# xarray-contrib/xeofs

Hardware: AMD Instinct MI355X
Metric: EOF randomized-SVD GB/s (algorithmic: 16 passes x n x p x 4 B per fit / fit time) (higher is better)
Workload: dtype f32 data, split-fp16 MFMA (f16x3+f16x3), f32 accumulate

## Files before the change

include/eofx.h:

```cpp
#ifndef EOFX_H
#define EOFX_H

#include <stdint.h>

#ifdef __cplusplus
extern "C" {
#endif

#define EOFX_ABI_VERSION 1
#define EOFX_MAX_SKETCH 256

#define EOFX_OK 0
#define EOFX_ERR_ARG (-1)
#define EOFX_ERR_HIP (-2)
#define EOFX_ERR_PARTIAL_NAN (-3)
#define EOFX_ERR_NAN_MISMATCH (-4)
#define EOFX_ERR_RANK (-5)
#define EOFX_ERR_LINALG (-6)
#define EOFX_ERR_NOMEM (-7)
#define EOFX_ERR_SHAPE (-8)

typedef struct eofx_ctx eofx_ctx;
typedef struct eofx_mat eofx_mat;

// ... 91 lines not shown
                           int n_oversamples, int n_iter, const float *omega, int flip, float *Q1,
                           float *s, float *Q2, float *scores1, float *scores2, float *norm1,
                           float *norm2, double *tsc);
typedef const float *(*eofx_sketch_fn)(void *user);
int eofx_crosscov_rsvd_lazy_f32(eofx_ctx *ctx, const eofx_mat *x, const eofx_mat *y, int k, int n_oversamples,
                                int n_iter, eofx_sketch_fn omega_fn, void *omega_user, int flip, float *Q1, float *s,
                                float *Q2, float *scores1, float *scores2, float *norm1, float *norm2, double *tsc);

int eofx_panel_tmul_f32(eofx_ctx *ctx, const eofx_mat *m, const float *Zn, float *Yp, int L,
                        int precision);
int eofx_panel_mul_f32(eofx_ctx *ctx, const eofx_mat *m, const float *Yp, float *Wn, int L,
                       int precision);
int eofx_panel_gram_f64(eofx_ctx *ctx, const float *P, int64_t rows_pad, int L, double *G);
int eofx_panel_cholqr_f32(eofx_ctx *ctx, const float *P, int64_t rows_pad, int L, int l,
                          const double *G, float *out);
int eofx_panel_rinv_f64(eofx_ctx *ctx, const double *G, int L, int l, double *Rinv);
int eofx_panel_matmul_f32(eofx_ctx *ctx, const float *P, int64_t rows_pad, int L,
                          const double *M, int Lo, float *out);
int eofx_panel_colminmax_f32(eofx_ctx *ctx, const float *P, int64_t rows, int L, float *mx,
                             float *mn);
int eofx_panel_export_f32(eofx_ctx *ctx, const float *P, int64_t rows, int L, int k,
                          const double *sign, float *dst);
int eofx_panel_import_f32(eofx_ctx *ctx, const float *src, int64_t rows, int l, float *P,
                          int64_t rows_pad, int L);

int eofx_hilbert_f32(eofx_ctx *ctx, const eofx_mat *a, int padding, double decay_factor,
                     eofx_mat **out_imag, eofx_mat **out_real);
int eofx_mat_sumsq_f64(eofx_ctx *ctx, const eofx_mat *m, double *out);
int eofx_panel_rownorm_f64(eofx_ctx *ctx, const float *P, int64_t rows, int L, double *out);
int eofx_mat_feature_norms_f64(eofx_ctx *ctx, const eofx_mat *m, double *out);
// ... 79 lines not shown
```

xeofs_amd/_lib.py:

```python

from __future__ import annotations

import ctypes as C
import os

import numpy as np

_HERE = os.path.dirname(os.path.abspath(__file__))
LIB_PATH = os.environ.get("EOFX_LIB") or os.path.join(_HERE, "lib", "libeofx.so")

EOFX_OK = 0
ERR_ARG, ERR_HIP, ERR_PARTIAL_NAN, ERR_NAN_MISMATCH, ERR_RANK, ERR_LINALG, ERR_NOMEM, ERR_SHAPE = (
    -1, -2, -3, -4, -5, -6, -7, -8)

_vp = C.c_void_p
_i64 = C.c_int64
_int = C.c_int
_pi64 = C.POINTER(C.c_int64)
_pd = C.POINTER(C.c_double)

SKETCH_FN = C.CFUNCTYPE(C.c_void_p, C.c_void_p)

ALLREDUCE_FN = C.CFUNCTYPE(C.c_int, C.c_void_p, C.c_void_p, C.c_int64, C.c_int, C.c_int, C.c_void_p)

# ... 15 lines not shown
    "eofx_mat_from_dense_f32": (_int, [_vp, _vp, _i64, _i64, _i64, C.POINTER(_vp)]),
    "eofx_mat_destroy": (_int, [_vp, _vp]),
    "eofx_mat_shape": (_int, [_vp, _pi64, _pi64, _pi64, _pi64]),
    "eofx_mat_download_f32": (_int, [_vp, _vp, _vp]),
    "eofx_rsvd_f32": (_int, [_vp, _vp, _int, _int, _int, _vp, _int, _vp, _vp, _vp]),
    "eofx_project_f32": (_int, [_vp, _vp, _vp, _int, _vp]),
    "eofx_reconstruct_f32": (_int, [_vp, _vp, _vp, _i64, _i64, _int, _vp]),
    "eofx_crosscov_rsvd_f32": (_int, [_vp, _vp, _vp, _int, _int, _int, _vp, _int, _vp, _vp, _vp, _vp,
                                      _vp, _vp, _vp, _pd]),
    "eofx_crosscov_rsvd_lazy_f32": (_int, [_vp, _vp, _vp, _int, _int, _int, SKETCH_FN, _vp, _int, _vp, _vp, _vp, _vp,
                                           _vp, _vp, _vp, _pd]),
    "eofx_panel_tmul_f32": (_int, [_vp, _vp, _vp, _vp, _int, _int]),
    "eofx_panel_mul_f32": (_int, [_vp, _vp, _vp, _vp, _int, _int]),
    "eofx_panel_gram_f64": (_int, [_vp, _vp, _i64, _int, _vp]),
    "eofx_panel_cholqr_f32": (_int, [_vp, _vp, _i64, _int, _int, _vp, _vp]),
    "eofx_panel_rinv_f64": (_int, [_vp, _vp, _int, _int, _vp]),
    "eofx_panel_matmul_f32": (_int, [_vp, _vp, _i64, _int, _vp, _int, _vp]),
    "eofx_panel_colminmax_f32": (_int, [_vp, _vp, _i64, _int, _vp, _vp]),
    "eofx_panel_export_f32": (_int, [_vp, _vp, _i64, _int, _int, _vp, _vp]),
    "eofx_panel_import_f32": (_int, [_vp, _vp, _i64, _int, _vp, _i64, _int]),
    "eofx_hilbert_f32": (_int, [_vp, _vp, _int, C.c_double, C.POINTER(_vp), C.POINTER(_vp)]),
    "eofx_mat_sumsq_f64": (_int, [_vp, _vp, _pd]),
    "eofx_fit_f32": (_int, [_vp, _vp, _i64, _i64, _int, _int, _vp, _int, _int, _int, _int, _vp, _i64, _int,
                            C.POINTER(_vp), _vp, _vp, _vp, _vp, _pi64, _pi64, _pd, _vp, _vp, _vp, C.POINTER(C.c_int)]),
    "eofx_fit_first_f32": (_int, [_vp, _vp, _i64, _i64, _int, _int, _vp, _int, _vp, _int, _int, _vp, C.POINTER(_vp),
                                  _vp, _vp, _vp, _vp, _pi64, _pi64, _pd, C.POINTER(C.c_int)]),
    "eofx_ctx_fit_info": (_int, [_vp, _pd]),
    "eofx_ctx_last_iterations": (_int, [_vp, C.POINTER(_int)]),
    "eofx_comm_unique_id": (_int, [C.c_char_p]),
    "eofx_ctx_comm_init_rccl": (_int, [_vp, C.c_char_p, _int, _int]),
# ... 117 lines not shown
```

xeofs_amd/csrc/eofx_abi.hip:

```cpp
#include <chrono>
#include "eofx_hfft.hpp"
#include "eofx_kernels.hpp"
#include "eofx_fit.hpp"
#include "eofx_gram.hpp"
#include "eofx_axb_dma.hpp"
#include "eofx_hosteig.hpp"
#include "eofx_hostla.hpp"
#include "eofx_lag.hpp"
#include "eofx_gw.hpp"
#include "eofx_spca.hpp"
#include "eofx_lagcov.hpp"
#include "eofx_lowpass.hpp"
#include "eofx_pcmul.hpp"
#include "eofx_viewcov.hpp"
#include "eofx_lrfill.hpp"
#include "eofx_plans.hpp"
#include "eofx_sketch.hpp"
#include "eofx_hilbert_host.hpp"
#include "eofx_gwplan.hpp"
#ifndef EOFX_AXB_DMA_DEFAULT
#define EOFX_AXB_DMA_DEFAULT 1
#endif

#include <algorithm>
// ... 708 lines not shown
  }
  if (plan.S > 1) {
    const int64_t count4 = rows_pad * L / 4;
    hipLaunchKernelGGL(splitk_reduce_kernel, dim3((int)std::min<int64_t>((count4 + 255) / 256, amax_out ? 2048 : 4096)), dim3(256), 0,
                       ctx->stream, out, W, count4, plan.S, amax_out);
    KCHK();
  }
  return EOFX_OK;
}

static int launch_gram(eofx_ctx* ctx, const float* P, int64_t rows, int L, double* G) {
  const int nb = (L + 63) / 64;
  const int nbx = gram_parts(rows, L);
  ArenaScope scope(ctx);
  ARENA(double, part, (size_t)nbx * L * L);
  hipLaunchKernelGGL(gram_mfma_kernel, dim3(nbx, nb * nb), dim3(256), 0, ctx->stream, P, rows, L, part);
  KCHK();
  const int64_t count = (int64_t)L * L;
  hipLaunchKernelGGL(f64_reduce_kernel, dim3((int)((count + 63) / 64)), dim3(256), 0, ctx->stream,
                     part, G, count, nbx);
  KCHK();
  return EOFX_OK;
}
static int launch_matmul(eofx_ctx* ctx, const float* P, int64_t rows, int L, const double* Mx, int Lo,
                         float* out, bool upper = false) {
  int KW = (int)std::min<int64_t>(round_up(L, 64), 256);
  if (L > 256) {
    static const int kw_env = std::getenv("EOFX_PMM_KW") ? atoi(std::getenv("EOFX_PMM_KW")) : 0;
    if (kw_env == 128 || kw_env == 256) KW = kw_env;
  }
  const size_t smem = (size_t)KW * PMM_LD * sizeof(double);
  if (smem > 64 * 1024)
    HIPCHK(hipFuncSetAttribute(reinterpret_cast<const void*>(panel_matmul_kernel<false>), hipFuncAttributeMaxDynamicSharedMemorySize, (int)smem));
  const int64_t units = (rows + 127) / 128;
  const int64_t gx = L <= KW ? std::min<int64_t>(units, 1024) : units;
  dim3 grid((int)std::max<int64_t>(1, gx), (Lo + 63) / 64);
  hipLaunchKernelGGL(panel_matmul_kernel<false>, grid, dim3(256), smem, ctx->stream, P, rows, L, Mx, Lo, out, KW, amax_new(ctx, out),
                     (int64_t)0, (int64_t)0, 1, (const float*)nullptr, upper ? 1 : 0);
  KCHK();
  return EOFX_OK;
}
static int launch_matmul_gen(eofx_ctx* ctx, const float* P, int64_t ldp, int64_t slab, int cpb, int64_t rows, int L, const double* Mx, int Lo,
                             const float* sub, float* out) {
  const int KW = (int)std::min<int64_t>(round_up(L, 64), 256);
  const size_t smem = (size_t)KW * PMM_LD * sizeof(double);
  if (smem > 64 * 1024)
    HIPCHK(hipFuncSetAttribute(reinterpret_cast<const void*>(panel_matmul_kernel<true>), hipFuncAttributeMaxDynamicSharedMemorySize, (int)smem));
  const int64_t units = (rows + 127) / 128;
  const int64_t gx = L <= KW ? std::min<int64_t>(units, 1024) : units;
  dim3 grid((int)std::max<int64_t>(1, gx), (Lo + 63) / 64);
  hipLaunchKernelGGL(panel_matmul_kernel<true>, grid, dim3(256), smem, ctx->stream, P, rows, L, Mx, Lo, out, KW, amax_new(ctx, out), ldp,
                     slab, cpb, sub);
  KCHK();
// ... 7 lines not shown
  KCHK();
  const int64_t count = (int64_t)La * Lb;
  hipLaunchKernelGGL(f64_reduce_kernel, dim3((int)((count + 63) / 64)), dim3(256), 0, ctx->stream, part, C, count, nbx);
  KCHK();
  return EOFX_OK;
}

static int launch_rinv(eofx_ctx* ctx, const double* G, int L, int l, double* Rinv);
static size_t matmul_nt_scratch(eofx_ctx* ctx, int64_t rows, int L, int Lo);
static int launch_matmul_nt(eofx_ctx* ctx, const float* P, int64_t rows, int L, const double* Mx, int Lo, float* out);
static int launch_cholqr(eofx_ctx* ctx, const float* P, int64_t rows, int L, int l, const double* G,
                         float* out) {
  ArenaScope scope(ctx);
  ARENA(double, Rinv, (size_t)L * L);
  CHK(launch_rinv(ctx, G, L, l, Rinv));
  return launch_matmul(ctx, P, rows, L, Rinv, L, out, true);
}

static int launch_colminmax(eofx_ctx* ctx, const float* P, int64_t rows, int L, float* mx, float* mn) {
  const int nparts = (int)std::max<int64_t>(1, std::min<int64_t>((rows + 127) / 128, 1024));
  ArenaScope scope(ctx);
  ARENA(float, pmx, (size_t)nparts * L);
  ARENA(float, pmn, (size_t)nparts * L);
  hipLaunchKernelGGL(colminmax_part_kernel, dim3(nparts, (L + 63) / 64), dim3(256), 0, ctx->stream, P,
                     rows, L, pmx, pmn);
  KCHK();
  hipLaunchKernelGGL(colminmax_final_kernel, dim3((L + 63) / 64), dim3(256), 0, ctx->stream, pmx, pmn,
                     nparts, L, mx, mn);
  KCHK();
  return EOFX_OK;
}
// ... 806 lines not shown
  return panel_mul(ctx, m, Yp, Wn, L, prec);
}
extern "C" int eofx_panel_gram_f64(eofx_ctx* ctx, const float* P, int64_t rows_pad, int L, double* G) {
  if (!ctx || !P || !G || L % 32) return set_err(ctx, EOFX_ERR_ARG, "bad argument");
  ENTER(ctx);
  CHK(arena_reserve(ctx, (size_t)(4 * gram_parts(rows_pad, L) + 1) * L * L * sizeof(double)));
  return launch_gram(ctx, P, rows_pad, L, G);
}
extern "C" int eofx_panel_cholqr_f32(eofx_ctx* ctx, const float* P, int64_t rows_pad, int L, int l,
                                     const double* G, float* out) {
  if (!ctx || !P || !G || !out || P == out) return set_err(ctx, EOFX_ERR_ARG, "bad argument");
  ENTER(ctx);
  CHK(arena_reserve(ctx, (size_t)2 * L * L * sizeof(double) + (l > 64 ? rinv_blocked_bytes(l) : 0)));
  return launch_cholqr(ctx, P, rows_pad, L, l, G, out);
}
extern "C" int eofx_panel_rinv_f64(eofx_ctx* ctx, const double* G, int L, int l, double* Rinv) {
  if (!ctx || !G || !Rinv || L <= 0 || l <= 0 || l > L || G == Rinv) return set_err(ctx, EOFX_ERR_ARG, "bad argument");
  ENTER(ctx);
  if (l > 64) CHK(arena_reserve(ctx, rinv_blocked_bytes(l)));
  return launch_rinv(ctx, G, L, l, Rinv);
}
extern "C" int eofx_panel_matmul_f32(eofx_ctx* ctx, const float* P, int64_t rows_pad, int L,
                                     const double* M, int Lo, float* out) {
  if (!ctx || !P || !M || !out || P == out) return set_err(ctx, EOFX_ERR_ARG, "bad argument");
  ENTER(ctx);
  if (matmul_nt_ok(rows_pad, L, Lo)) {
    const size_t need = matmul_nt_scratch(ctx, rows_pad, L, Lo);
    if (need && arena_reserve(ctx, need) == EOFX_OK) return launch_matmul_nt(ctx, P, rows_pad, L, M, Lo, out);
  }
  return launch_matmul(ctx, P, rows_pad, L, M, Lo, out);
// ... 27 lines not shown
struct LinOp {
  int64_t tall, small, tall_pad, small_pad;
  std::function<int(const float*, float*, int, int)> fwd;
  std::function<int(const float*, float*, int, int)> bwd;
  std::function<int(double*, int64_t)> reduce_tall_gram;
  std::function<int(double*, int64_t)> reduce_small_gram;
  int64_t rule_tall_pad = 0;
};

struct RsvdOut {
  float* Tvec;
  float* Svec;
  int Lo;
  std::vector<double> s;
  int64_t tall_pad = 0, small_pad = 0;
};

extern "C" int eofx_orth_tall_rule(int64_t tall_rows_pad, int L, int prec_power) {
  return orth_tall_rule(tall_rows_pad, L, prec_power) ? 1 : 0;
}
extern "C" int eofx_peaked_spectrum(const double* G, int ld, int l) {
  if (!G || l <= 0) return 0;
  std::vector<double> A((size_t)l * l), w(l), V((size_t)l * l);
  for (int i = 0; i < l; ++i)
    for (int j = 0; j < l; ++j) A[(size_t)i * l + j] = 0.5 * (G[(size_t)i * ld + j] + G[(size_t)j * ld + i]);
  for (double v : A)
    if (!std::isfinite(v)) return 0;
  if (eofx_host_eigh_f64(A.data(), l, w.data(), V.data()) != EOFX_OK) return 1;
  if (!(w[0] > 0.0)) return 0;
  return hostla::peaked_spectrum(w.data(), l) ? 1 : 0;
// ... 155 lines not shown
        rc = set_err(ctx, EOFX_ERR_HIP, "asynchronous Gram download failed");
        break;
      }
      peaked_pending = true;
    }
    rc = launch_cholqr(ctx, Ws, op.small_pad, L, l, ask ? G0 : G, Zs);
  }
  if (peaked_ev) {
    if (peaked_pending) (void)hipEventSynchronize(peaked_ev);
    (void)hipEventDestroy(peaked_ev);
  }
  if (rc != EOFX_OK) return rc;
  if (range) CHK((*range)(Zs, Yt, L));
  else CHK(fwd(Zs, Yt, pp));
  CHK(gram_tall(Yt, G));
  CHK(launch_cholqr(ctx, Yt, op.tall_pad, L, l, G, Qt));
  CHK(gram_tall(Qt, G));
  CHK(launch_rinv(ctx, G, L, l, R2));
  CHK(op.bwd(Qt, Zs, L, pf));
  CHK(launch_matmul(ctx, Zs, op.small_pad, L, R2, L, Ws));
  CHK(gram_small(Ws, G));
  double* hG = pin;
  double* hR2 = pin + (size_t)L * L;
  HIPCHK(hipMemcpyAsync(hG, G, sizeof(double) * L * L, hipMemcpyDeviceToHost, ctx->stream));
  HIPCHK(hipMemcpyAsync(hR2, R2, sizeof(double) * L * L, hipMemcpyDeviceToHost, ctx->stream));
  HIPCHK(hipStreamSynchronize(ctx->stream));
  std::vector<double> Gl((size_t)l * l), w(l), Uh((size_t)l * l);
  for (int i = 0; i < l; ++i)
    for (int j = 0; j < l; ++j) {
      const double v = 0.5 * (hG[(size_t)i * L + j] + hG[(size_t)j * L + i]);
      if (!std::isfinite(v))
        return set_err(ctx, EOFX_ERR_LINALG,
// ... 8 lines not shown
    const double sv = std::sqrt(std::max(w[j], 0.0));
    out.s[j] = sv;
    invs[j] = sv > 0.0 ? 1.0 / sv : 0.0;
  }
  for (int i = 0; i < l; ++i) {
    double* m1 = &M1[(size_t)i * Lo];
    for (int q = 0; q < l; ++q) {
      const double r = hR2[(size_t)i * L + q];
      const double* uq = &Uh[(size_t)q * l];
      for (int j = 0; j < k; ++j) m1[j] += r * uq[j];
    }
    for (int j = 0; j < k; ++j) M2[(size_t)i * Lo + j] = Uh[(size_t)i * l + j] * invs[j];
  }
  HIPCHK(hipMemcpyAsync(Md, M1.data(), sizeof(double) * L * Lo, hipMemcpyHostToDevice, ctx->stream));
  HIPCHK(hipMemcpyAsync(Md2, M2.data(), sizeof(double) * L * Lo, hipMemcpyHostToDevice, ctx->stream));
  CHK(launch_matmul(ctx, Qt, op.tall_pad, L, Md, Lo, Tv));
  CHK(launch_matmul(ctx, Ws, op.small_pad, L, Md2, Lo, Sv));
  HIPCHK(hipStreamSynchronize(ctx->stream));
  out.Tvec = Tv;
  out.Svec = Sv;
  out.Lo = Lo;
  out.tall_pad = op.tall_pad;
  out.small_pad = op.small_pad;
  return EOFX_OK;
}

static int comm_allreduce(eofx_ctx* ctx, void* buf, int64_t count, int dtype, int op);
static int sign_rule(eofx_ctx* ctx, const float* Vpanel, int64_t rows, int Lo, int k,
                     std::vector<double>& sign, bool over_ranks = false) {
  ArenaScope scope(ctx);
  ARENA(float, mx, 2 * (size_t)Lo);
  float* mn = mx + Lo;
  CHK(launch_colminmax(ctx, Vpanel, rows, Lo, mx, mn));
  if (over_ranks) {
    hipLaunchKernelGGL(negate_kernel, dim3(1), dim3(256), 0, ctx->stream, mn, Lo);
    KCHK();
    CHK(comm_allreduce(ctx, mx, 2 * (int64_t)Lo, 0, 1));
  }
  std::vector<float> hmx(Lo), hmn(Lo);
  HIPCHK(hipMemcpyAsync(hmx.data(), mx, sizeof(float) * Lo, hipMemcpyDeviceToHost, ctx->stream));
  HIPCHK(hipMemcpyAsync(hmn.data(), mn, sizeof(float) * Lo, hipMemcpyDeviceToHost, ctx->stream));
  HIPCHK(hipStreamSynchronize(ctx->stream));
  sign.assign(k, 1.0);
  for (int j = 0; j < k; ++j) sign[j] = (std::fabs(hmx[j]) >= std::fabs(hmn[j])) ? 1.0 : -1.0;
  return EOFX_OK;
}

typedef std::function<int(double*, int64_t)> GramReduce;
// ... 35 lines not shown
      CHK(refill());
      continue;
    }
    HIPCHK(hipMemcpyAsync(Mx, hM.data(), sizeof(double) * Lo * Lo, hipMemcpyHostToDevice, ctx->stream));
    CHK(launch_matmul(ctx, P, rows_pad, Lo, Mx, Lo, tmp));
    HIPCHK(hipMemcpy2DAsync(P + first, sizeof(float) * Lo, tmp + first, sizeof(float) * Lo, sizeof(float) * (size_t)(k - first), (size_t)rows_pad,
                            hipMemcpyDeviceToDevice, ctx->stream));
    HIPCHK(hipStreamSynchronize(ctx->stream));
    ++rounds_done;
  }
  return EOFX_OK;
}

static int fix_null_modes(eofx_ctx* ctx, const RsvdOut& ro, int64_t tall, int64_t small, int k,
                          const GramReduce* reduce_tall = nullptr, int64_t tall_total = -1,
                          const GramReduce* reduce_small = nullptr, int64_t small_total = -1) {
  int first_null = k;
  const double s0 = ro.s.empty() ? 0.0 : ro.s[0];
  for (int j = k - 1; j >= 0 && !(ro.s[j] > 1e-5 * s0); --j) first_null = j;
  if (first_null < k && s0 >= 0.0 && std::isfinite(s0) && ro.tall_pad >= tall && ro.small_pad >= small) {
    CHK(fix_null_columns(ctx, ro.Tvec, tall, ro.tall_pad, ro.Lo, k, first_null, reduce_tall, tall_total));
    CHK(fix_null_columns(ctx, ro.Svec, small, ro.small_pad, ro.Lo, k, first_null, reduce_small, small_total));
  }
  return EOFX_OK;
}

struct FactorShards {
  const GramReduce* reduce_tall = nullptr;
  int64_t tall_total = -1;
  const GramReduce* reduce_small = nullptr;
  int64_t small_total = -1;
};
static int rsvd_finish(eofx_ctx* ctx, const RsvdOut& ro, bool right_is_tall, int64_t left_rows, int64_t right_rows, int k, int flip,
                       float* left, float* s, float* right, double s_divisor = 1.0, const FactorShards* shards = nullptr,
                       std::vector<double>* sign_out = nullptr) {
  const int64_t tall = right_is_tall ? right_rows : left_rows, small = right_is_tall ? left_rows : right_rows;
  const FactorShards local, &sh = shards ? *shards : local;
  CHK(fix_null_modes(ctx, ro, tall, small, k, sh.reduce_tall, sh.tall_total, sh.reduce_small, sh.small_total));
  const float* Rp = right_is_tall ? ro.Tvec : ro.Svec;
  const float* Lp = right_is_tall ? ro.Svec : ro.Tvec;
  std::vector<double> sign;
  if (flip) CHK(sign_rule(ctx, Rp, right_rows, ro.Lo, k, sign, shards != nullptr));
  CHK(export_panel(ctx, Lp, left_rows, ro.Lo, k, flip ? sign.data() : nullptr, left));
  CHK(export_panel(ctx, Rp, right_rows, ro.Lo, k, flip ? sign.data() : nullptr, right));
  if (s) {
    std::vector<float> hs(k);
    for (int j = 0; j < k; ++j) hs[j] = (float)(ro.s[j] / s_divisor);
    HIPCHK(hipMemcpy(s, hs.data(), sizeof(float) * k, hipMemcpyDefault));
  }
  HIPCHK(hipStreamSynchronize(ctx->stream));
  if (sign_out) sign_out->swap(sign);
  return EOFX_OK;
}

static const float* identity_sketch(int64_t small, int l, std::vector<float>& eye) {
  eye.assign((size_t)small * l, 0.f);
  for (int64_t i = 0; i < l; ++i) eye[(size_t)i * l + i] = 1.f;
// ... 3122 lines not shown
```

xeofs_amd/csrc/eofx_kernels.hpp:

```cpp
#pragma once
#include <hip/hip_runtime.h>
#include <stdint.h>

#include "eofx_mfma64.hpp"
#include "eofx_plans.hpp"

namespace eofx {

typedef float f32x16 __attribute__((ext_vector_type(16)));
typedef float f32x4 __attribute__((ext_vector_type(4)));
typedef float f32x2 __attribute__((ext_vector_type(2)));

__device__ __forceinline__ void aff_split(double sh, float& hi, float& lo) {
  hi = (float)sh;
  lo = (float)(sh - (double)hi);
}
__device__ __forceinline__ float aff_map(float x, float sh_hi, float sh_lo, float scale) {
  return ((x - sh_hi) - sh_lo) * scale;
}
__device__ __forceinline__ float aff_fma(float x, float sh_hi, float s, float nls) {
  return __builtin_fmaf(x - sh_hi, s, nls);
}

__device__ __forceinline__ void amax_commit(float mx, unsigned* __restrict__ amax_out) {
// ... 1008 lines not shown
                                }
                              });
    __syncthreads();
  }
  double* G = Gpart + (int64_t)blockIdx.x * (int64_t)L * L;
  for (int e = threadIdx.x; e < 64 * 64; e += 256) {
    const int i = e >> 6, j = e & 63;
    const int gi = 64 * bi + i, gj = 64 * bj + j;
    if (gi < L && gj < L) {
      G[(int64_t)gi * L + gj] = Gs[i][j];
      if (!same) G[(int64_t)gj * L + gi] = Gs[i][j];
    }
  }
}

__global__ __launch_bounds__(256) void f64_reduce_kernel(const double* __restrict__ part,
                                                         double* __restrict__ out, int64_t count,
                                                         int nparts) {
  __shared__ double red[4][64];
  const int li = threadIdx.x & 63, q = threadIdx.x >> 6;
  const int64_t i = (int64_t)blockIdx.x * 64 + li;
  double s = 0;
  if (i < count) {
#pragma unroll 4
    for (int b = q; b < nparts; b += 4) s += part[(int64_t)b * count + i];
  }
  red[q][li] = s;
  __syncthreads();
  if (q == 0 && i < count) out[i] = ((red[0][li] + red[1][li]) + red[2][li]) + red[3][li];
}
// ... 269 lines not shown
    if (r < l && c < l) v = G[(int64_t)r * L + c];
    S[i] = v;
    if (r == c) d0[r] = v;
  }
}
__global__ void chol_blocked_export_kernel(const double* __restrict__ X, int Lb, int l, double* __restrict__ Rinv, int L) {
  const int64_t total = (int64_t)L * L;
  for (int64_t i = (int64_t)blockIdx.x * blockDim.x + threadIdx.x; i < total; i += (int64_t)gridDim.x * blockDim.x) {
    const int r = (int)(i / L), c = (int)(i % L);
    Rinv[i] = (r <= c && c < l) ? X[(int64_t)r * Lb + c] : 0.0;
  }
}

constexpr int PMM_LD = 66;

template <bool GEN = false>
__global__ __launch_bounds__(256) void panel_matmul_kernel(const float* __restrict__ P,
                                                           int64_t rows, int L,
                                                           const double* __restrict__ Mx, int Lo,
                                                           float* __restrict__ out, int KW,
                                                           unsigned* __restrict__ amax_out = nullptr,
                                                           int64_t ldp = 0, int64_t slab = 0, int cpb = 1,
                                                           const float* __restrict__ sub = nullptr, int upper = 0) {
  extern __shared__ __attribute__((aligned(16))) double Ms[];
  float amx = 0.f;
  const int tid = threadIdx.x;
  const int lane = tid & 63, wave = tid >> 6;
  const int li = lane & 15, lk = lane >> 4;
  const int by = upper ? (int)(gridDim.y - 1 - blockIdx.y) : (int)blockIdx.y;
  const int c0 = by * 64;
  const int Lc_all = (L + 63) / 64;
  const int Lc = upper ? (Lc_all < by + 1 ? Lc_all : by + 1) : Lc_all;
  const int Le = L < 64 * Lc ? L : 64 * Lc;
  const int64_t ngroups = (rows + 31) / 32;
  const int64_t g0 = (int64_t)blockIdx.x * 4 + wave;
  auto stage = [&](int k0) {
    for (int i = tid; i < KW * 64; i += 256) {
      const int r = i >> 6, c = i & 63;
// ... 5 lines not shown
    for (int t = 0; t < 2; ++t) {
      const int64_t r = 32 * g + 16 * t + li;
#pragma unroll
      for (int tt = 0; tt < 4; ++tt) {
        const int k = kc + 16 * tt + 4 * lk;
        if constexpr (GEN)
          a[t][tt] = (valid && r < rows && k < L) ? *reinterpret_cast<const f32x4*>(P + (int64_t)((k >> 6) / cpb) * slab + ((k >> 6) % cpb) * 64 + r * ldp + (k & 63))
                                                 : f32x4{0.f, 0.f, 0.f, 0.f};
        else
          a[t][tt] = (valid && r < rows && k < L) ? *reinterpret_cast<const f32x4*>(P + r * L + k)
                                                 : f32x4{0.f, 0.f, 0.f, 0.f};
      }
    }
  };
  f64x4 acc[2][4];
  auto compute = [&](int64_t g, int kc, int ms0, const f32x4 (&a)[2][4]) {
    if (kc == 0) {
#pragma unroll
      for (int t = 0; t < 2; ++t)
#pragma unroll
        for (int q = 0; q < 4; ++q) acc[t][q] = f64x4{0.0, 0.0, 0.0, 0.0};
    }
#pragma unroll
    for (int tt = 0; tt < 4; ++tt)
#pragma unroll
      for (int c = 0; c < 4; ++c) {
        double b[4];
#pragma unroll
        for (int q = 0; q < 4; ++q) b[q] = Ms[(kc - ms0 + 16 * tt + 4 * lk + c) * PMM_LD + 16 * q + li];
#pragma unroll
// ... 7 lines not shown
      for (int t = 0; t < 2; ++t)
#pragma unroll
        for (int r = 0; r < 4; ++r) {
          const int64_t row = 32 * g + 16 * t + lk + 4 * r;
          if (row >= rows) continue;
#pragma unroll
          for (int q = 0; q < 4; ++q) {
            const int col = c0 + 16 * q + li;
            if (col < Lo) {
              float o_ = (float)acc[t][q][r];
              if constexpr (GEN) {
                if (sub) o_ = (float)((double)sub[row * Lo + col] - acc[t][q][r]);
              }
              out[row * Lo + col] = o_;
              amx = fmaxf(amx, fabsf(o_));
            }
          }
        }
    }
  };
  f32x4 a0[2][4], a1[2][4];
  if (Lc * 64 <= KW) {
    stage(0);
    __syncthreads();
    const int64_t gstride = (int64_t)gridDim.x * 4;
    const int64_t nitems = g0 < ngroups ? ((ngroups - g0 + gstride - 1) / gstride) * Lc : 0;
    fetch(nitems > 0, g0, 0, a0);
    for (int64_t item = 0; item < nitems; item += 2) {
      fetch(item + 1 < nitems, g0 + ((item + 1) / Lc) * gstride, (int)((item + 1) % Lc) * 64, a1);
      __builtin_amdgcn_sched_barrier(0);
// ... 12 lines not shown
      __syncthreads();
      stage(64 * w0);
      __syncthreads();
      const int we = w0 + wc < Lc ? w0 + wc : Lc;
      for (int ch = w0; ch < we; ch += 2) {
        fetch(active && ch + 1 < Lc, g0, 64 * (ch + 1), a1);
        __builtin_amdgcn_sched_barrier(0);
        if (active) compute(g0, 64 * ch, 64 * w0, a0);
        fetch(active && ch + 2 < Lc, g0, 64 * (ch + 2), a0);
        __builtin_amdgcn_sched_barrier(0);
        if (active && ch + 1 < we) compute(g0, 64 * (ch + 1), 64 * w0, a1);
      }
    }
  }
  if (amax_out) amax_commit(amx, amax_out);
}

__global__ __launch_bounds__(256) void colminmax_part_kernel(const float* __restrict__ P,
                                                             int64_t rows, int L,
                                                             float* __restrict__ pmx,
                                                             float* __restrict__ pmn) {
  __shared__ float smx[16][64], smn[16][64];
  const int tid = threadIdx.x;
  const int cq = tid & 15, rl = tid >> 4;
  const int c = blockIdx.y * 64 + 4 * cq;
  f32x4 mx = {-INFINITY, -INFINITY, -INFINITY, -INFINITY}, mn = {INFINITY, INFINITY, INFINITY, INFINITY};
  if (c < L) {
    const int64_t step = (int64_t)gridDim.x * 16;
    int64_t r = (int64_t)blockIdx.x * 16 + rl;
    for (; r + 7 * step < rows; r += 8 * step) {
// ... 1132 lines not shown
```

xeofs_amd/engine.py:

```python

from __future__ import annotations

import contextlib
import ctypes as C
import numbers

import numpy as np

from . import _lib
from ._lib import ptr, raise_for


def _f32c(a):
    if isinstance(a, np.ndarray):
        return np.ascontiguousarray(a, dtype=np.float32)
    if hasattr(a, "data_ptr"):
        import torch

        if a.dtype != torch.float32 or not a.is_contiguous():
            a = a.to(torch.float32).contiguous()
        return a
    return np.ascontiguousarray(np.asarray(a), dtype=np.float32)


# ... 733 lines not shown
    torch = _torch()
    L = P.shape[1]
    if out is None:
        out = torch.empty((L, L), dtype=torch.float64, device=P.device)
    raise_for(ctx.lib.eofx_panel_gram_f64(ctx.handle, ptr(P), P.shape[0], L, ptr(out)), ctx.handle)
    return out


def panel_cholqr(ctx: Context, P, l: int, G, out=None):
    torch = _torch()
    if out is None:
        out = torch.empty_like(P)
    raise_for(ctx.lib.eofx_panel_cholqr_f32(ctx.handle, ptr(P), P.shape[0], P.shape[1], int(l), ptr(G), ptr(out)),
              ctx.handle)
    return out


def panel_rinv(ctx: Context, G, l: int):
    torch = _torch()
    out = torch.empty_like(G)
    raise_for(ctx.lib.eofx_panel_rinv_f64(ctx.handle, ptr(G), G.shape[0], int(l), ptr(out)), ctx.handle)
    return out


def panel_matmul(ctx: Context, P, M, out=None):
    torch = _torch()
    Lo = M.shape[1]
    if out is None:
        out = torch.empty((P.shape[0], Lo), dtype=torch.float32, device=P.device)
    raise_for(ctx.lib.eofx_panel_matmul_f32(ctx.handle, ptr(P), P.shape[0], P.shape[1], ptr(M), Lo, ptr(out)),
# ... 510 lines not shown
```

Measured before the change: 6043.

## Fuse CholQR with re-Gram and column min/max into panel matmul kernels

Adds a fused panel_matmul_gram kernel that applies R^-1 and accumulates the Gram of the resulting Q in one pass, replacing the separate cholqr and gram passes over the tall panel when L <= 64. It also adds a single-tile diagonal Gram kernel for narrow panels, and fuses per-block column min/max into the final tall projection matmul so the sign rule only reduces partials. The goal is to cut full re-reads of the tall panel in exchange for more register pressure and extra code paths. A tall Gram reduce callback is now invoked explicitly after the fused step.

```diff
diff --git a/include/eofx.h b/include/eofx.h
--- a/include/eofx.h
+++ b/include/eofx.h
@@ -129,6 +129,8 @@
 int eofx_panel_gram_f64(eofx_ctx *ctx, const float *P, int64_t rows_pad, int L, double *G);
 int eofx_panel_cholqr_f32(eofx_ctx *ctx, const float *P, int64_t rows_pad, int L, int l,
                           const double *G, float *out);
+int eofx_panel_cholqr_gram_f32(eofx_ctx *ctx, const float *P, int64_t rows_pad, int L, int l, const double *G,
+                               float *Q_out, double *G2_out);
 int eofx_panel_rinv_f64(eofx_ctx *ctx, const double *G, int L, int l, double *Rinv);
 int eofx_panel_matmul_f32(eofx_ctx *ctx, const float *P, int64_t rows_pad, int L,
                           const double *M, int Lo, float *out);
diff --git a/xeofs_amd/_lib.py b/xeofs_amd/_lib.py
--- a/xeofs_amd/_lib.py
+++ b/xeofs_amd/_lib.py
@@ -53,6 +53,7 @@
     "eofx_panel_mul_f32": (_int, [_vp, _vp, _vp, _vp, _int, _int]),
     "eofx_panel_gram_f64": (_int, [_vp, _vp, _i64, _int, _vp]),
     "eofx_panel_cholqr_f32": (_int, [_vp, _vp, _i64, _int, _int, _vp, _vp]),
+    "eofx_panel_cholqr_gram_f32": (_int, [_vp, _vp, _i64, _int, _int, _vp, _vp, _vp]),
     "eofx_panel_rinv_f64": (_int, [_vp, _vp, _int, _int, _vp]),
     "eofx_panel_matmul_f32": (_int, [_vp, _vp, _i64, _int, _vp, _int, _vp]),
     "eofx_panel_colminmax_f32": (_int, [_vp, _vp, _i64, _int, _vp, _vp]),
diff --git a/xeofs_amd/csrc/eofx_abi.hip b/xeofs_amd/csrc/eofx_abi.hip
--- a/xeofs_amd/csrc/eofx_abi.hip
+++ b/xeofs_amd/csrc/eofx_abi.hip
@@ -746,7 +746,10 @@
   const int nbx = gram_parts(rows, L);
   ArenaScope scope(ctx);
   ARENA(double, part, (size_t)nbx * L * L);
-  hipLaunchKernelGGL(gram_mfma_kernel, dim3(nbx, nb * nb), dim3(256), 0, ctx->stream, P, rows, L, part);
+  if (nb == 1)
+    hipLaunchKernelGGL(gram_diag_mfma_kernel, dim3(nbx), dim3(64 * GRAM_DIAG_WAVES), 0, ctx->stream, P, rows, L, part);
+  else
+    hipLaunchKernelGGL(gram_mfma_kernel, dim3(nbx, nb * nb), dim3(256), 0, ctx->stream, P, rows, L, part);
   KCHK();
   const int64_t count = (int64_t)L * L;
   hipLaunchKernelGGL(f64_reduce_kernel, dim3((int)((count + 63) / 64)), dim3(256), 0, ctx->stream,
@@ -754,8 +757,14 @@
   KCHK();
   return EOFX_OK;
 }
+struct ColExtrema {
+  float *pmx = nullptr, *pmn = nullptr;
+  int parts = 0;
+  int64_t rows = 0;
+};
+constexpr int PMM_MAX_GRID = 1024;
 static int launch_matmul(eofx_ctx* ctx, const float* P, int64_t rows, int L, const double* Mx, int Lo,
-                         float* out, bool upper = false) {
+                         float* out, bool upper = false, ColExtrema* ext = nullptr) {
   int KW = (int)std::min<int64_t>(round_up(L, 64), 256);
   if (L > 256) {
     static const int kw_env = std::getenv("EOFX_PMM_KW") ? atoi(std::getenv("EOFX_PMM_KW")) : 0;
@@ -765,10 +774,17 @@
   if (smem > 64 * 1024)
     HIPCHK(hipFuncSetAttribute(reinterpret_cast<const void*>(panel_matmul_kernel<false>), hipFuncAttributeMaxDynamicSharedMemorySize, (int)smem));
   const int64_t units = (rows + 127) / 128;
-  const int64_t gx = L <= KW ? std::min<int64_t>(units, 1024) : units;
+  const int64_t gx = L <= KW ? std::min<int64_t>(units, PMM_MAX_GRID) : units;
   dim3 grid((int)std::max<int64_t>(1, gx), (Lo + 63) / 64);
-  hipLaunchKernelGGL(panel_matmul_kernel<false>, grid, dim3(256), smem, ctx->stream, P, rows, L, Mx, Lo, out, KW, amax_new(ctx, out),
-                     (int64_t)0, (int64_t)0, 1, (const float*)nullptr, upper ? 1 : 0);
+  if (ext && L <= KW && smem <= 64 * 1024) {
+    ext->parts = (int)grid.x;
+    hipLaunchKernelGGL((panel_matmul_kernel<false, true>), grid, dim3(256), smem, ctx->stream, P, rows, L, Mx, Lo, out, KW, amax_new(ctx, out),
+                       (int64_t)0, (int64_t)0, 1, (const float*)nullptr, upper ? 1 : 0, ext->pmx, ext->pmn, ext->rows);
+  } else {
+    if (ext) ext->parts = 0;
+    hipLaunchKernelGGL(panel_matmul_kernel<false>, grid, dim3(256), smem, ctx->stream, P, rows, L, Mx, Lo, out, KW, amax_new(ctx, out),
+                       (int64_t)0, (int64_t)0, 1, (const float*)nullptr, upper ? 1 : 0, (float*)nullptr, (float*)nullptr, (int64_t)0);
+  }
   KCHK();
   return EOFX_OK;
 }
@@ -806,7 +822,34 @@
   ArenaScope scope(ctx);
   ARENA(double, Rinv, (size_t)L * L);
   CHK(launch_rinv(ctx, G, L, l, Rinv));
+  if (L <= 64) {
+    const int64_t units = (rows + 127) / 128;
+    hipLaunchKernelGGL(panel_matmul_gram_kernel<false>, dim3((int)std::max<int64_t>(1, std::min<int64_t>(units, PMM_MAX_GRID))), dim3(256),
+                       (size_t)64 * PMM_LD * sizeof(double), ctx->stream, P, rows, L, (const double*)Rinv, out, (double*)nullptr,
+                       amax_new(ctx, out));
+    KCHK();
+    return EOFX_OK;
+  }
   return launch_matmul(ctx, P, rows, L, Rinv, L, out, true);
+}
+
+static int launch_cholqr_gram(eofx_ctx* ctx, const float* P, int64_t rows, int L, int l, const double* G, float* out, double* G2) {
+  if (L > 64) {
+    CHK(launch_cholqr(ctx, P, rows, L, l, G, out));
+    return launch_gram(ctx, out, rows, L, G2);
+  }
+  const int nparts = gram_parts(rows, L);
+  ArenaScope scope(ctx);
+  ARENA(double, Rinv, (size_t)L * L);
+  ARENA(double, part, (size_t)nparts * L * L);
+  CHK(launch_rinv(ctx, G, L, l, Rinv));
+  hipLaunchKernelGGL(panel_matmul_gram_kernel<true>, dim3(nparts), dim3(256), (size_t)64 * PMM_LD * sizeof(double), ctx->stream, P, rows, L,
+                     (const double*)Rinv, out, part, amax_new(ctx, out));
+  KCHK();
+  const int64_t count = (int64_t)L * L;
+  hipLaunchKernelGGL(f64_reduce_kernel, dim3((int)((count + 63) / 64)), dim3(256), 0, ctx->stream, (const double*)part, G2, count, nparts);
+  KCHK();
+  return EOFX_OK;
 }
 
 static int launch_colminmax(eofx_ctx* ctx, const float* P, int64_t rows, int L, float* mx, float* mn) {
@@ -1643,6 +1686,14 @@
   CHK(arena_reserve(ctx, (size_t)2 * L * L * sizeof(double) + (l > 64 ? rinv_blocked_bytes(l) : 0)));
   return launch_cholqr(ctx, P, rows_pad, L, l, G, out);
 }
+extern "C" int eofx_panel_cholqr_gram_f32(eofx_ctx* ctx, const float* P, int64_t rows_pad, int L, int l, const double* G, float* Q_out,
+                                          double* G2_out) {
+  if (!ctx || !P || !G || !Q_out || !G2_out || P == Q_out || L <= 0 || L % 32 || l <= 0 || l > L || rows_pad < 0)
+    return set_err(ctx, EOFX_ERR_ARG, "bad argument");
+  ENTER(ctx);
+  CHK(arena_reserve(ctx, (size_t)(4 * gram_parts(rows_pad, L) + 3) * L * L * sizeof(double) + (l > 64 ? rinv_blocked_bytes(l) : 0)));
+  return launch_cholqr_gram(ctx, P, rows_pad, L, l, G, Q_out, G2_out);
+}
 extern "C" int eofx_panel_rinv_f64(eofx_ctx* ctx, const double* G, int L, int l, double* Rinv) {
   if (!ctx || !G || !Rinv || L <= 0 || l <= 0 || l > L || G == Rinv) return set_err(ctx, EOFX_ERR_ARG, "bad argument");
   ENTER(ctx);
@@ -1700,6 +1751,7 @@
   int Lo;
   std::vector<double> s;
   int64_t tall_pad = 0, small_pad = 0;
+  ColExtrema tall_ext;
 };
 
 extern "C" int eofx_orth_tall_rule(int64_t tall_rows_pad, int L, int prec_power) {
@@ -1885,8 +1937,8 @@
   if (range) CHK((*range)(Zs, Yt, L));
   else CHK(fwd(Zs, Yt, pp));
   CHK(gram_tall(Yt, G));
-  CHK(launch_cholqr(ctx, Yt, op.tall_pad, L, l, G, Qt));
-  CHK(gram_tall(Qt, G));
+  CHK(launch_cholqr_gram(ctx, Yt, op.tall_pad, L, l, G, Qt, G));
+  if (op.reduce_tall_gram) CHK(op.reduce_tall_gram(G, (int64_t)L * L));
   CHK(launch_rinv(ctx, G, L, l, R2));
   CHK(op.bwd(Qt, Zs, L, pf));
   CHK(launch_matmul(ctx, Zs, op.small_pad, L, R2, L, Ws));
@@ -1925,7 +1977,18 @@
   }
   HIPCHK(hipMemcpyAsync(Md, M1.data(), sizeof(double) * L * Lo, hipMemcpyHostToDevice, ctx->stream));
   HIPCHK(hipMemcpyAsync(Md2, M2.data(), sizeof(double) * L * Lo, hipMemcpyHostToDevice, ctx->stream));
-  CHK(launch_matmul(ctx, Qt, op.tall_pad, L, Md, Lo, Tv));
+  out.tall_ext = ColExtrema();
+  const size_t ext_floats = (size_t)PMM_MAX_GRID * Lo;
+  const size_t ext_keep_free = (size_t)std::max(op.tall_pad, op.small_pad) * (Lo + L) * 4 + ((size_t)2 << 20);
+  if (!std::getenv("EOFX_NO_FUSED_MINMAX") && 2 * ext_floats * sizeof(float) <= ((size_t)1 << 20) &&
+      ctx->arena_size - ctx->arena_off >= 2 * ext_floats * sizeof(float) + ext_keep_free) {
+    if (float* px = arena_alloc<float>(ctx, 2 * ext_floats)) {
+      out.tall_ext.pmx = px;
+      out.tall_ext.pmn = px + ext_floats;
+      out.tall_ext.rows = op.tall;
+    }
+  }
+  CHK(launch_matmul(ctx, Qt, op.tall_pad, L, Md, Lo, Tv, false, out.tall_ext.pmx ? &out.tall_ext : nullptr));
   CHK(launch_matmul(ctx, Ws, op.small_pad, L, Md2, Lo, Sv));
   HIPCHK(hipStreamSynchronize(ctx->stream));
   out.Tvec = Tv;
@@ -1938,11 +2001,17 @@
 
 static int comm_allreduce(eofx_ctx* ctx, void* buf, int64_t count, int dtype, int op);
 static int sign_rule(eofx_ctx* ctx, const float* Vpanel, int64_t rows, int Lo, int k,
-                     std::vector<double>& sign, bool over_ranks = false) {
+                     std::vector<double>& sign, bool over_ranks = false, const ColExtrema* ext = nullptr) {
   ArenaScope scope(ctx);
   ARENA(float, mx, 2 * (size_t)Lo);
   float* mn = mx + Lo;
-  CHK(launch_colminmax(ctx, Vpanel, rows, Lo, mx, mn));
+  if (ext) {
+    hipLaunchKernelGGL(colminmax_final_kernel, dim3((Lo + 63) / 64), dim3(256), 0, ctx->stream, (const float*)ext->pmx,
+                       (const float*)ext->pmn, ext->parts, Lo, mx, mn);
+    KCHK();
+  } else {
+    CHK(launch_colminmax(ctx, Vpanel, rows, Lo, mx, mn));
+  }
   if (over_ranks) {
     hipLaunchKernelGGL(negate_kernel, dim3(1), dim3(256), 0, ctx->stream, mn, Lo);
     KCHK();
@@ -2008,11 +2077,13 @@
 
 static int fix_null_modes(eofx_ctx* ctx, const RsvdOut& ro, int64_t tall, int64_t small, int k,
                           const GramReduce* reduce_tall = nullptr, int64_t tall_total = -1,
-                          const GramReduce* reduce_small = nullptr, int64_t small_total = -1) {
+                          const GramReduce* reduce_small = nullptr, int64_t small_total = -1, bool* repaired = nullptr) {
   int first_null = k;
   const double s0 = ro.s.empty() ? 0.0 : ro.s[0];
   for (int j = k - 1; j >= 0 && !(ro.s[j] > 1e-5 * s0); --j) first_null = j;
+  if (repaired) *repaired = false;
   if (first_null < k && s0 >= 0.0 && std::isfinite(s0) && ro.tall_pad >= tall && ro.small_pad >= small) {
+    if (repaired) *repaired = true;
     CHK(fix_null_columns(ctx, ro.Tvec, tall, ro.tall_pad, ro.Lo, k, first_null, reduce_tall, tall_total));
     CHK(fix_null_columns(ctx, ro.Svec, small, ro.small_pad, ro.Lo, k, first_null, reduce_small, small_total));
   }
@@ -2030,11 +2101,13 @@
                        std::vector<double>* sign_out = nullptr) {
   const int64_t tall = right_is_tall ? right_rows : left_rows, small = right_is_tall ? left_rows : right_rows;
   const FactorShards local, &sh = shards ? *shards : local;
-  CHK(fix_null_modes(ctx, ro, tall, small, k, sh.reduce_tall, sh.tall_total, sh.reduce_small, sh.small_total));
+  bool repaired = false;
+  CHK(fix_null_modes(ctx, ro, tall, small, k, sh.reduce_tall, sh.tall_total, sh.reduce_small, sh.small_total, &repaired));
   const float* Rp = right_is_tall ? ro.Tvec : ro.Svec;
   const float* Lp = right_is_tall ? ro.Svec : ro.Tvec;
   std::vector<double> sign;
-  if (flip) CHK(sign_rule(ctx, Rp, right_rows, ro.Lo, k, sign, shards != nullptr));
+  const bool ext_ok = right_is_tall && !repaired && ro.tall_ext.parts > 0 && ro.tall_ext.rows == right_rows;
+  if (flip) CHK(sign_rule(ctx, Rp, right_rows, ro.Lo, k, sign, shards != nullptr, ext_ok ? &ro.tall_ext : nullptr));
   CHK(export_panel(ctx, Lp, left_rows, ro.Lo, k, flip ? sign.data() : nullptr, left));
   CHK(export_panel(ctx, Rp, right_rows, ro.Lo, k, flip ? sign.data() : nullptr, right));
   if (s) {
diff --git a/xeofs_amd/csrc/eofx_kernels.hpp b/xeofs_amd/csrc/eofx_kernels.hpp
--- a/xeofs_amd/csrc/eofx_kernels.hpp
+++ b/xeofs_amd/csrc/eofx_kernels.hpp
@@ -1046,6 +1046,59 @@
   }
 }
 
+constexpr int GRAM_DIAG_WAVES = 8;
+constexpr int GRAM_DIAG_PF = 8;
+__global__ __launch_bounds__(64 * GRAM_DIAG_WAVES) void gram_diag_mfma_kernel(const float* __restrict__ P, int64_t rows, int L,
+                                                                               double* __restrict__ Gpart) {
+  const int wave = __builtin_amdgcn_readfirstlane(threadIdx.x >> 6);
+  const Mfma64Lane ln = mfma64_lane();
+  const int ca = 4 * ln.c;
+  const auto upper = [](int x, int y) { return y >= x; };
+  f64x4 acc[4][4];
+  mfma64_zero(acc);
+  const int64_t wstride = (int64_t)gridDim.x * GRAM_DIAG_WAVES * 4;
+  auto fetch = [&](int64_t r0, f32x4& va) {
+    const int64_t r = r0 + ln.k;
+    va = f32x4{0.f, 0.f, 0.f, 0.f};
+    if (r < rows && ca < L) va = *reinterpret_cast<const f32x4*>(P + r * L + ca);
+  };
+  int64_t r0 = ((int64_t)blockIdx.x * GRAM_DIAG_WAVES + wave) * 4;
+  f32x4 pa[GRAM_DIAG_PF];
+#pragma unroll
+  for (int d = 0; d < GRAM_DIAG_PF; ++d) fetch(r0 + d * wstride, pa[d]);
+  for (; r0 < rows; r0 += GRAM_DIAG_PF * wstride) {
+#pragma unroll
+    for (int d = 0; d < GRAM_DIAG_PF; ++d) {
+      const f32x4 va = pa[d];
+      fetch(r0 + (GRAM_DIAG_PF + d) * wstride, pa[d]);
+      __builtin_amdgcn_sched_barrier(0);
+      if (r0 + d * wstride < rows) {
+        const double a[4] = {(double)va[0], (double)va[1], (double)va[2], (double)va[3]};
+        mfma64_step(acc, a, a, upper);
+      }
+    }
+  }
+  __shared__ double Gs[64][65];
+  for (int w = 0; w < GRAM_DIAG_WAVES; ++w) {
+    if (wave == w)
+      mfma64_each_interleaved(acc, upper, [&](int x, int y, int i, int j, double v) {
+        if (w == 0) {
+          Gs[i][j] = v;
+          if (x < y) Gs[j][i] = v;
+        } else {
+          Gs[i][j] += v;
+          if (x < y) Gs[j][i] += v;
+        }
+      });
+    __syncthreads();
+  }
+  double* G = Gpart + (int64_t)blockIdx.x * (int64_t)L * L;
+  for (int e = threadIdx.x; e < 64 * 64; e += 64 * GRAM_DIAG_WAVES) {
+    const int i = e >> 6, j = e & 63;
+    if (i < L && j < L) G[(int64_t)i * L + j] = Gs[i][j];
+  }
+}
+
 __global__ __launch_bounds__(256) void f64_reduce_kernel(const double* __restrict__ part,
                                                          double* __restrict__ out, int64_t count,
                                                          int nparts) {
@@ -1345,14 +1398,16 @@
 
 constexpr int PMM_LD = 66;
 
-template <bool GEN = false>
+template <bool GEN = false, bool MINMAX = false>
 __global__ __launch_bounds__(256) void panel_matmul_kernel(const float* __restrict__ P,
                                                            int64_t rows, int L,
                                                            const double* __restrict__ Mx, int Lo,
                                                            float* __restrict__ out, int KW,
                                                            unsigned* __restrict__ amax_out = nullptr,
                                                            int64_t ldp = 0, int64_t slab = 0, int cpb = 1,
-                                                           const float* __restrict__ sub = nullptr, int upper = 0) {
+                                                           const float* __restrict__ sub = nullptr, int upper = 0,
+                                                           float* __restrict__ pmx = nullptr, float* __restrict__ pmn = nullptr,
+                                                           int64_t mm_rows = 0) {
   extern __shared__ __attribute__((aligned(16))) double Ms[];
   float amx = 0.f;
   const int tid = threadIdx.x;
@@ -1388,6 +1443,7 @@
     }
   };
   f64x4 acc[2][4];
+  float cmx[4] = {-INFINITY, -INFINITY, -INFINITY, -INFINITY}, cmn[4] = {INFINITY, INFINITY, INFINITY, INFINITY};
   auto compute = [&](int64_t g, int kc, int ms0, const f32x4 (&a)[2][4]) {
     if (kc == 0) {
 #pragma unroll
@@ -1425,6 +1481,12 @@
               }
               out[row * Lo + col] = o_;
               amx = fmaxf(amx, fabsf(o_));
+              if constexpr (MINMAX) {
+                if (row < mm_rows) {
+                  cmx[q] = fmaxf(cmx[q], o_);
+                  cmn[q] = fminf(cmn[q], o_);
+                }
+              }
             }
           }
         }
@@ -1467,6 +1529,132 @@
     }
   }
   if (amax_out) amax_commit(amx, amax_out);
+  if constexpr (MINMAX) {
+    __syncthreads();
+    float* smx = reinterpret_cast<float*>(Ms);
+    float* smn = smx + 16 * 64;
+#pragma unroll
+    for (int q = 0; q < 4; ++q) {
+      smx[(4 * wave + lk) * 64 + 16 * q + li] = cmx[q];
+      smn[(4 * wave + lk) * 64 + 16 * q + li] = cmn[q];
+    }
+    __syncthreads();
+    if (tid < 64 && c0 + tid < Lo) {
+      float a = smx[tid], b = smn[tid];
+      for (int s = 1; s < 16; ++s) {
+        a = fmaxf(a, smx[s * 64 + tid]);
+        b = fminf(b, smn[s * 64 + tid]);
+      }
+      pmx[(int64_t)blockIdx.x * Lo + c0 + tid] = a;
+      pmn[(int64_t)blockIdx.x * Lo + c0 + tid] = b;
+    }
+  }
+}
+
+template <bool GRAM>
+__global__ __launch_bounds__(256) void panel_matmul_gram_kernel(const float* __restrict__ P, int64_t rows, int L,
+                                                                const double* __restrict__ Mx, float* __restrict__ out,
+                                                                double* __restrict__ Gpart,
+                                                                unsigned* __restrict__ amax_out = nullptr) {
+  extern __shared__ __attribute__((aligned(16))) double Ms[];
+  float amx = 0.f;
+  const int tid = threadIdx.x;
+  const int lane = tid & 63, wave = __builtin_amdgcn_readfirstlane(tid >> 6);
+  const int li = lane & 15, lk = lane >> 4;
+  const int64_t ngroups = (rows + 31) / 32;
+  const int64_t g0 = (int64_t)blockIdx.x * 4 + wave;
+  for (int i = tid; i < 64 * 64; i += 256) {
+    const int r = i >> 6, c = i & 63;
+    Ms[r * PMM_LD + c] = (r < L && c < L) ? Mx[(int64_t)r * L + c] : 0.0;
+  }
+  auto fetch = [&](bool valid, int64_t g, f32x4 (&a)[2][4]) {
+#pragma unroll
+    for (int t = 0; t < 2; ++t) {
+      const int64_t r = 32 * g + 16 * t + li;
+#pragma unroll
+      for (int tt = 0; tt < 4; ++tt) {
+        const int k = 16 * tt + 4 * lk;
+        a[t][tt] = (valid && r < rows && k < L) ? *reinterpret_cast<const f32x4*>(P + r * L + k) : f32x4{0.f, 0.f, 0.f, 0.f};
+      }
+    }
+  };
+  f64x4 gacc[4][4];
+  mfma64_zero(gacc);
+  const auto upper = [](int x, int y) { return y >= x; };
+  auto compute = [&](int64_t g, const f32x4 (&a)[2][4]) {
+    f64x4 acc[2][4];
+    mfma64_zero(acc);
+#pragma unroll
+    for (int tt = 0; tt < 4; ++tt)
+#pragma unroll
+      for (int c = 0; c < 4; ++c) {
+        double b[4];
+#pragma unroll
+        for (int q = tt; q < 4; ++q) b[q] = Ms[(16 * tt + 4 * lk + c) * PMM_LD + 16 * q + li];
+#pragma unroll
+        for (int t = 0; t < 2; ++t)
+#pragma unroll
+          for (int q = tt; q < 4; ++q)
+            acc[t][q] = __builtin_amdgcn_mfma_f64_16x16x4f64((double)a[t][tt][c], b[q], acc[t][q], 0, 0, 0);
+      }
+#pragma unroll
+    for (int t = 0; t < 2; ++t)
+#pragma unroll
+      for (int r = 0; r < 4; ++r) {
+        const int64_t row = 32 * g + 16 * t + lk + 4 * r;
+        double o[4];
+#pragma unroll
+        for (int q = 0; q < 4; ++q) {
+          const int col = 16 * q + li;
+          const float o_ = (float)acc[t][q][r];
+          o[q] = (double)o_;
+          if (row < rows && col < L) {
+            out[row * L + col] = o_;
+            amx = fmaxf(amx, fabsf(o_));
+          }
+        }
+        if constexpr (GRAM) mfma64_step(gacc, o, o, upper);
+      }
+  };
+  __syncthreads();
+  constexpr int NBUF = GRAM ? 4 : 2;
+  f32x4 a[NBUF][2][4];
+  const int64_t gstride = (int64_t)gridDim.x * 4;
+  const int64_t nitems = g0 < ngroups ? (ngroups - g0 + gstride - 1) / gstride : 0;
+#pragma unroll
+  for (int d = 0; d < NBUF - 1; ++d) fetch(d < nitems, g0 + d * gstride, a[d]);
+  for (int64_t item = 0; item < nitems; item += NBUF) {
+#pragma unroll
+    for (int d = 0; d < NBUF; ++d) {
+      if (item + d < nitems) {
+        fetch(item + d + NBUF - 1 < nitems, g0 + (item + d + NBUF - 1) * gstride, a[(d + NBUF - 1) % NBUF]);
+        __builtin_amdgcn_sched_barrier(0);
+        compute(g0 + (item + d) * gstride, a[d]);
+      }
+    }
+  }
+  if (amax_out) amax_commit(amx, amax_out);
+  if constexpr (GRAM) {
+    __syncthreads();
+    for (int w = 0; w < 4; ++w) {
+      if (wave == w)
+        mfma64_each_blocked(gacc, upper, [&](int x, int y, int i, int j, double v) {
+          if (w == 0) {
+            Ms[i * PMM_LD + j] = v;
+            if (x < y) Ms[j * PMM_LD + i] = v;
+          } else {
+            Ms[i * PMM_LD + j] += v;
+            if (x < y) Ms[j * PMM_LD + i] += v;
+          }
+        });
+      __syncthreads();
+    }
+    double* G = Gpart + (int64_t)blockIdx.x * (int64_t)L * L;
+    for (int e = tid; e < 64 * 64; e += 256) {
+      const int i = e >> 6, j = e & 63;
+      if (i < L && j < L) G[(int64_t)i * L + j] = Ms[i * PMM_LD + j];
+    }
+  }
 }
 
 __global__ __launch_bounds__(256) void colminmax_part_kernel(const float* __restrict__ P,
diff --git a/xeofs_amd/engine.py b/xeofs_amd/engine.py
--- a/xeofs_amd/engine.py
+++ b/xeofs_amd/engine.py
@@ -771,6 +771,17 @@
     raise_for(ctx.lib.eofx_panel_cholqr_f32(ctx.handle, ptr(P), P.shape[0], P.shape[1], int(l), ptr(G), ptr(out)),
               ctx.handle)
     return out
+
+
+def panel_cholqr_gram(ctx: Context, P, l: int, G, out=None, G2=None):
+    torch = _torch()
+    if out is None:
+        out = torch.empty_like(P)
+    if G2 is None:
+        G2 = torch.empty_like(G)
+    raise_for(ctx.lib.eofx_panel_cholqr_gram_f32(ctx.handle, ptr(P), P.shape[0], P.shape[1], int(l), ptr(G), ptr(out),
+                                                 ptr(G2)), ctx.handle)
+    return out, G2
 
 
 def panel_rinv(ctx: Context, G, l: int):
```

After: 5896. 0.976x the previous value.
